# wendongbi/Bridged-GNN

Hardware: AMD Instinct MI355X
Metric: aggregated_edges_per_sec_ktgnn_fwd (higher is better)
Workload: dtype f32; 1 GPU; C4 synthetic bridged graph (local) N=1000000 E'=20991058, 2-layer KT-GNN eval fwd F=128 hidden=128 C=2; parallelism=single, execution=eager launches

## Files before the change

bridged_gnn_amd/_lib.py:

```python
import ctypes as C
import os

import torch

_HERE = os.path.dirname(os.path.abspath(__file__))
SO_PATH = os.path.join(_HERE, "csrc", "libbgnn_hip.so")
_lib = None

_P, _I64, _I32, _F32, _SZ, _INT = C.c_void_p, C.c_int64, C.c_int32, C.c_float, C.c_size_t, C.c_int

SIGNATURES = {
    "bgnn_version": (_INT, []),
    "bgnn_source_hash": (C.c_char_p, []),
    "bgnn_error_string": (C.c_char_p, [_INT]),
    "bgnn_csr_workspace_bytes": (_SZ, [_I64, _I64]),
    "bgnn_build_dst_csr": (_INT, [_P, _I64, _I64, _INT, _P, _P, _P, _P, _P, _SZ, _P]),
    "bgnn_domain_sums_f64": (_INT, [_P, _I64, _I32, _I64, _P, _P, _P]),
    "bgnn_domain_sums_workspace_bytes": (_SZ, [_I32]),
    "bgnn_domain_sums_ws_f64": (_INT, [_P, _I64, _I32, _I64, _P, _P, _P, _SZ, _P]),
    "bgnn_domain_delta_f32": (_INT, [_P, _I32, _P, _P]),
    "bgnn_adaptedconv_transform_f32": (_INT, [_P, _I64, _I32, _I64, _P, _P, _P, _I32, _I32, _P, _P, _P, _P,
                                               _P, _P, _P, _P, _I64, _I64, _I64, _I64, _P, _P, _I32, _P, _P]),
    "bgnn_classifier_stage_f32": (_INT, [_P, _I64, _I32, _I64, _P, _P, _I32, _I32, _P, _P, _P, _P, _P, _P, _P, _P, _I64, _I64,
                                          _P, _P, _I32, _INT, _P, _P, _P, _P, _P, _P]),
# ... 4 lines not shown
    "bgnn_narrow_transform_finish_rows32_f32": (_INT, [_P, _I64, _P, _P, _I32, _P, _P, _P, _P, _P, _P, _I64, _P, _P]),
    "bgnn_adaptedconv_aggregate_heads_rows32_plan": (_INT, [_P, _P, _I64, _I64, _I32, _F32]),
    "bgnn_adaptedconv_aggregate_heads_rows32_f32": (_INT, [_P, _P, _P, _P, _P, _P, _P, _I64, _I64, _I32, _F32, _P, _INT, _I64, _P]),
    "bgnn_gram_workspace_bytes": (C.c_size_t, [_I32, _I32]),
    "bgnn_gram_f32": (_INT, [_P, _I64, _I32, _P, _I64, _I32, _I64, _P, _P, C.c_size_t, _P]),
    "bgnn_transform_bwd_prep_workspace_bytes": (C.c_size_t, [_I64, _I32]),
    "bgnn_transform_bwd_prep_f32": (_INT, [_P, _I64, _I64, _I32, _P, _P, _I64, _I32, _P, _P, _P, _P, _P, _P, _I32, _I64, _P, _I64, _P, _P, C.c_size_t, _P]),
    "bgnn_bn_acc_doubles": (_I64, [_I32]),
    "bgnn_bn_relu_dropout_f32": (_INT, [_P, _I64, _I32, _I64, _P, _P, _F32, _INT, _F32, C.c_uint64, _P, _F32, _P, _P, _P, _I64, _P, _P]),
    "bgnn_bn_relu_dropout_bwd_f32": (_INT, [_P, _P, _I64, _I32, _I64, _I64, _P, _P, _P, _F32, _INT, _F32, C.c_uint64, _P, _P, _I64, _P, _P]),
    "bgnn_bn_colstats_f32": (_INT, [_P, _I64, _I32, _I64, _P, _P]),
    "bgnn_bn_apply_rows_f32": (_INT, [_P, _I64, _I32, _I64, _P, _I64, _P, _P, _F32, _INT, _F32, C.c_uint64, _P, _P, _I64, _F32, _P, _P, _P, _I64, _P]),
    "bgnn_bn_bwd_reduce_rows_f32": (_INT, [_P, _P, _I64, _I32, _I64, _I64, _P, _I64, _P, _P, _F32, _INT, _F32, C.c_uint64, _P, _P, _I64, _P, _P]),
    "bgnn_bn_bwd_apply_rows_f32": (_INT, [_P, _P, _I64, _I32, _I64, _I64, _P, _P, _I64, _P, _P, _F32, _INT, _F32, C.c_uint64, _P, _P, _I64, _P, _I64, _P]),
    "bgnn_transform_bwd_consts_f32": (_INT, [_P, _P, _P, _P, _P, _I32, _I32, _P, _P, _P, _P]),
    "bgnn_transform_bwd_finish_f32": (_INT, [_P, _P, _P, _P, _P, _P, _P, _I32, _I32, _I32, _P, _P, _P, _P, _P, _P, _P, _I64, _P]),
    "bgnn_rowdot_f32": (_INT, [_P, _I64, _I64, _I32, _P, _I64, _I32, _P, _P]),
    "bgnn_linear_f32": (_INT, [_P, _I64, _I32, _I64, _P, _P, _I32, _INT, _P, _P, _P, _I64, _P]),
    "bgnn_adaptedconv_aggregate_f32": (_INT, [_P, _P, _I64, _P, _P, _P, _P, _P, _I64, _I64, _I32, _F32,
                                               _P, _I64, _P, _P, _P, _INT, _P, _INT, _I64, _I32, _P, _P, _P]),
    "bgnn_adaptedconv_aggregate_bounded_f32": (_INT, [_P, _P, _I64, _P, _P, _P, _P, _P, _I64, _I64, _I32, _F32,
                                                       _P, _I64, _P, _P, _P, _INT, _P, _INT, _I64, _I32, _P, _P, _I64, _I32, _P]),
    "bgnn_aggregate_tile_queue_words": (_I64, []),
    "bgnn_adaptedconv_aggregate_queued_f32": (_INT, [_P, _P, _I64, _P, _P, _P, _P, _P, _I64, _I64, _I32, _F32,
                                                      _P, _I64, _P, _P, _P, _INT, _P, _INT, _I64, _I32, _P, _P, _I64, _I64, _I32, _P]),
    "bgnn_aggregate_hub_workspace_bytes": (C.c_size_t, [_I64, _I32, _I64]),
    "bgnn_adaptedconv_aggregate_hub_f32": (_INT, [_P, _P, _I64, _P, _P, _P, _P, _P, _I64, _I32, _F32, _P, _I64, _P, _P, _INT, _P, _I32, _P,
                                                   _P, _I32, _P, _I64, _P, _P, _P, _I64, _P, _P, C.c_size_t, _P]),
    "bgnn_adaptedconv_aggregate_bwd_f32": (_INT, [_P, _P, _I64, _P, _P, _P, _P, _P, _I64, _I64, _I32, _F32,
                                                   _P, _I64, _P, _P, _I64, _P, _P, _P, _P, _P]),
    "bgnn_aggregate_bwd_pull_workspace_bytes": (C.c_size_t, [_I64, _I64, _I64, _I32, _I64, _I64]),
    "bgnn_adaptedconv_aggregate_bwd_pull_f32": (_INT, [_P, _P, _I64, _P, _P, _P, _P, _P, _P, _P, _P, _I64, _I64, _I32, _F32,
                                                        _P, _I64, _P, _P, _I64, _P, _P, _P, _P, _I32,
                                                        _P, _I64, _P, _P, _P, _I64, _P, _I64, _P, _P, _P, _I64, _P, C.c_size_t, _P]),
    "bgnn_aggregate_heads_bwd_workspace_bytes": (C.c_size_t, [_I64, _I64, _I32, _I64, _I64]),
    "bgnn_adaptedconv_aggregate_heads_bwd_f32": (_INT, [_P, _P, _P, _P, _P, _P, _P, _P, _P, _I64, _I64, _I32, _I32, _F32,
                                                         _P, _P, _P, _INT, _P, _P, _P, _P, _I32,
                                                         _P, _I64, _P, _P, _P, _I64, _P, _I64, _P, _P, _P, _I64, _P, C.c_size_t, _P]),
    "bgnn_adaptedconv_aggregate_heads_wide_f32": (_INT, [_P, _P, _I64, _P, _P, _P, _P, _P, _I64, _I32, _I32, _F32, _P, _P, _P]),
    "bgnn_aggregate_heads_wide_bwd_workspace_bytes": (C.c_size_t, [_I64, _I32, _I64]),
    "bgnn_adaptedconv_aggregate_heads_wide_bwd_f32": (_INT, [_P, _P, _I64, _P, _P, _P, _P, _P, _P, _P, _I64, _I32, _I32, _F32,
                                                              _P, _P, _P, _P, _P, _P, _P, _P, C.c_size_t, _P]),
    "bgnn_l2_normalize_rows_f32": (_INT, [_P, _I64, _I32, _F32, _P, _P]),
    "bgnn_topk_workspace_bytes": (_SZ, [_I64, _I64, _I32]),
    "bgnn_cosine_topk_f32": (_INT, [_P, _P, _I64, _I64, _I32, _I32, _INT, _P, _P, _P, _P, _SZ, _P]),
    "bgnn_mlp_pair_topk_f32": (_INT, [_P, _P, _P, _P, _P, _F32, _I64, _I64, _I32, _I32, _INT, _P, _P, _P,
# ... 210 lines not shown
```

bridged_gnn_amd/csrc/bgnn_aggregate.hip:

```cpp
#include <cstdlib>
#include <cstring>
#include <type_traits>
#include "bgnn_common.h"

namespace {

struct AggParams {
  const float* h_t2s;
  const float* h_s2t;
  int64_t ldh;
  const float* a_t2s;
  const float* a_s2t;
  const int32_t* rowptr;
  const int32_t* col;
  const uint8_t* mask;
  int64_t row_begin;
  int64_t row_end;
  int32_t D;
  float slope;
  float* out;
  int64_t ldo;
  float* alpha;
  const float* ep_scale;
  const float* ep_shift;
// ... 479 lines not shown
  }
  if (p.colsum != nullptr) {
    unsafeAtomicAdd(&red[0][f0], cs_s.x); unsafeAtomicAdd(&red[0][f0 + 1], cs_s.y);
    unsafeAtomicAdd(&red[0][f0 + 2], cs_s.z); unsafeAtomicAdd(&red[0][f0 + 3], cs_s.w);
    unsafeAtomicAdd(&red[1][f0], cs_t.x); unsafeAtomicAdd(&red[1][f0 + 1], cs_t.y);
    unsafeAtomicAdd(&red[1][f0 + 2], cs_t.z); unsafeAtomicAdd(&red[1][f0 + 3], cs_t.w);
    if (lg == 0) { unsafeAtomicAdd(&red[0][LF * 4], n_s); unsafeAtomicAdd(&red[1][LF * 4], n_t); }
    __syncthreads();
    for (int t = threadIdx.x; t < 2 * (LF * 4 + 1); t += 256) {
      const int d = t / (LF * 4 + 1), c = t % (LF * 4 + 1);
      const double sum = (double)red[d][c];
      if (c == LF * 4) unsafeAtomicAdd(&p.colsum[2 * p.ldo + d], sum);
      else if (c < p.ldo) unsafeAtomicAdd(&p.colsum[d * p.ldo + c], sum);
    }
  }
}

typedef unsigned int u32x4_t __attribute__((ext_vector_type(4)));
constexpr int TQ_SPACING_WORDS = 32;

template <int CTRL>
__device__ __forceinline__ uint32_t dpp_movu(uint32_t x) { return (uint32_t)__builtin_amdgcn_update_dpp(0, (int)x, CTRL, 0xF, 0xF, true); }

template <int LF, bool ALPHA>
__global__ __launch_bounds__(256) void agg_wide_fast_kernel(AggParams p) {
  static_assert(LF == 16 || LF == 32 || LF == 64, "wide rows only");
  constexpr int U = 4;
  constexpr int GPW = 64 / LF;
  constexpr int RPB = 4 * GPW;
  const int lane = threadIdx.x & 63;
  const int wave = threadIdx.x >> 6;
  const int g = lane / LF;
  const int lg = lane % LF;
  const int f0 = lg * 4;
  const bool fvalid = f0 < p.D;
  const int f0c = fvalid ? f0 : 0;
  const int k = lane & (U - 1);
  const bool b0 = lane & 1, b1 = lane & 2;

  const int32_t row0 = (int32_t)p.row_begin, row1 = (int32_t)p.row_end;
  const int32_t ntiles = (row1 - row0 + RPB - 1) / RPB;
  __shared__ float red[2][LF * 4 + 1];
  __shared__ unsigned long long cl_ring[4];
  __shared__ uint32_t cl_prog[4];
  const bool tile_claims = p.tile_queue != nullptr && p.tq_subqueues > 0;
  if (tile_claims && threadIdx.x < 4) { cl_ring[threadIdx.x] = 0ull; cl_prog[threadIdx.x] = 0u; }
  if (p.colsum != nullptr)
    for (int t = threadIdx.x; t < 2 * (LF * 4 + 1); t += 256) (&red[0][0])[t] = 0.f;
  if (p.colsum != nullptr || tile_claims) __syncthreads();
  __shared__ unsigned int dyn_tile;
  const uint32_t nstride = (uint32_t)(p.ldh * 4);
  const uint32_t ostride = (uint32_t)(p.ldo * 4);
  const __amdgpu_buffer_rsrc_t rt = __builtin_amdgcn_make_buffer_rsrc(const_cast<char*>(p.tbl_base), (short)0, (int)p.tbl_bytes, 0x00020000);
  const __amdgpu_buffer_rsrc_t ro = __builtin_amdgcn_make_buffer_rsrc(p.out, (short)0, (int)((uint32_t)row1 * ostride), 0x00020000);
  const f2 sl = {p.slope, p.slope};
  float sc4[4] = {0.f, 0.f, 0.f, 0.f}, sh4[4] = {0.f, 0.f, 0.f, 0.f};
  if (p.ep_scale != nullptr) {
#pragma unroll
    for (int c = 0; c < 4; ++c)
      if (f0 + c < p.D) { sc4[c] = p.ep_scale[f0 + c]; sh4[c] = p.ep_shift[f0 + c]; }
  }
  f2 cs_s01 = {0.f, 0.f}, cs_s23 = cs_s01, cs_t01 = cs_s01, cs_t23 = cs_s01;
  float n_s = 0.f, n_t = 0.f;
  f2 aS01 = {0.f, 0.f}, aS23 = aS01, aT01 = aS01, aT23 = aS01;
  if (fvalid) {
    aS01.x = p.a_t2s[f0]; aS01.y = f0 + 1 < p.D ? p.a_t2s[f0 + 1] : 0.f;
    aS23.x = f0 + 2 < p.D ? p.a_t2s[f0 + 2] : 0.f; aS23.y = f0 + 3 < p.D ? p.a_t2s[f0 + 3] : 0.f;
    aT01.x = p.a_s2t[f0]; aT01.y = f0 + 1 < p.D ? p.a_s2t[f0 + 1] : 0.f;
    aT23.x = f0 + 2 < p.D ? p.a_s2t[f0 + 2] : 0.f; aT23.y = f0 + 3 < p.D ? p.a_s2t[f0 + 3] : 0.f;
  }
  const int32_t TQ_CHUNK = p.tq_chunk;
  const int32_t xcd = blockIdx.x % 8, slot = blockIdx.x / 8;
  const int32_t G = ((int32_t)gridDim.x + 7 - xcd) / 8;
  const int32_t tstride = p.tq_interleave ? G : 1;
  const int32_t NSEG = p.xcd_segments > 1 ? p.xcd_segments : 1;
  const int32_t per_x = (ntiles + 7) / 8, seg_len = (per_x + NSEG - 1) / NSEG;
  const int32_t xbase = xcd * per_x;
  const int32_t xend = NSEG > 1 ? xbase + NSEG * seg_len : min((xcd + 1) * per_x, ntiles);
  int32_t tile = xbase + slot - G;
  int32_t chunk_left = 0;
  const int32_t NQ = tile_claims ? min((int32_t)p.tq_subqueues, G) : 0;
  const int32_t wave_u = __builtin_amdgcn_readfirstlane(wave);
  uint32_t* const qctr = NQ > 0 ? p.tile_queue + (xcd * NQ + slot % NQ) * TQ_SPACING_WORDS : nullptr;
  const int32_t qpos0 = xbase + (NQ > 0 ? slot % NQ : 0);
  uint32_t cl_n = 0;
  uint32_t cl_val = 0;
  bool cl_own = false, cl_pending = false;
  bool cl_ending = false, cl_stop = false;
  auto cl_issue = [&](uint32_t& v) {
    uint64_t ex;
    asm volatile("s_mov_b64 %1, exec\n\ts_mov_b64 exec, 1\n\tglobal_atomic_add %0, %2, %3, %4 sc0\n\ts_mov_b64 exec, %1"
                 : "+v"(v), "=&s"(ex) : "v"(0u), "v"(1u), "s"(qctr) : "memory");
  };
// ... 63 lines not shown
      if (tile >= xend) break;
    }
    int32_t gt = tile;
    if (NSEG > 1) {
      const int32_t j = tile - xbase, sg = j / seg_len;
      gt = (sg * 8 + xcd) * seg_len + (j - sg * seg_len);
      if (gt >= ntiles) {
        if (cl_own) {
          uint32_t v = 0;
          cl_issue(v);
          cl_wait(v);
          cl_publish(cl_n + 1u, v);
        }
        continue;
      }
    }
    const int32_t i0 = row0 + gt * RPB + wave * GPW + g;
    const bool rvalid = i0 < row1;
    const int32_t ic = rvalid ? i0 : row0;
    const bool dom_s = p.mask[ic] != 0;
    const int32_t beg = rvalid ? p.rowptr[ic] : 0;
    const int32_t end = rvalid ? p.rowptr[ic + 1] : 0;
    const uint32_t lbase = (dom_s ? p.off_t2s : p.off_s2t) + (uint32_t)f0c * 4u;
    const f2 a01 = dom_s ? aS01 : aT01, a23 = dom_s ? aS23 : aT23;
    const float4 hi4 = __builtin_bit_cast(float4, __builtin_amdgcn_raw_buffer_load_b128(rt, lbase + __umul24((uint32_t)ic, nstride), 0, 0));
    f2 h01 = {hi4.x, hi4.y}, h23 = {hi4.z, hi4.w};

    float m = -INFINITY, s = 0.f;
    f2 acc01 = {0.f, 0.f}, acc23 = {0.f, 0.f};
    const int32_t niter = (end - beg + U - 1) / U;
    auto issue = [&](float4 (&v)[U], uint32_t off) {
      v[0] = __builtin_bit_cast(float4, __builtin_amdgcn_raw_buffer_load_b128(rt, lbase + dpp_movu<0x00>(off), 0, 0));
      v[1] = __builtin_bit_cast(float4, __builtin_amdgcn_raw_buffer_load_b128(rt, lbase + dpp_movu<0x55>(off), 0, 0));
      v[2] = __builtin_bit_cast(float4, __builtin_amdgcn_raw_buffer_load_b128(rt, lbase + dpp_movu<0xAA>(off), 0, 0));
      v[3] = __builtin_bit_cast(float4, __builtin_amdgcn_raw_buffer_load_b128(rt, lbase + dpp_movu<0xFF>(off), 0, 0));
      asm volatile("" : "+v"(h01), "+v"(h23) : : "memory");
      __builtin_amdgcn_sched_barrier(0);
    };
    auto take_id = [&](uint32_t& id) {
      __builtin_amdgcn_sched_barrier(0);
      asm volatile("s_waitcnt vmcnt(0)" : "+v"(id), "+v"(m), "+v"(s), "+v"(acc01), "+v"(acc23) : : "memory");
    };
    auto load_id = [&](int32_t ee) {
      uint32_t id;
      const uint32_t eoff = (uint32_t)max(min(ee, end - 1), 0) * 4u;
      __builtin_amdgcn_sched_barrier(0);
      asm volatile("global_load_dword %0, %1, %2" : "=v"(id) : "v"(eoff), "s"(p.col) : "memory");
      __builtin_amdgcn_sched_barrier(0);
      return id;
    };
    auto row_off = [&](uint32_t id, bool alive) { return alive ? __umul24(id, nstride) : p.dead_off; };
    auto update = [&](const float4 (&v)[U], bool ok, int32_t e_cur) {
      float t[U];
#pragma unroll
      for (int u = 0; u < U; ++u) {
        f2 z0 = f2{v[u].x, v[u].y} + h01, z1 = f2{v[u].z, v[u].w} + h23;
        z0 = __builtin_elementwise_max(z0, z0 * sl);
        z1 = __builtin_elementwise_max(z1, z1 * sl);
        f2 q = a01 * z0;
        q = __builtin_elementwise_fma(a23, z1, q);
        t[u] = q.x + q.y;
      }
      const float rA = bfly<0xB1>(b0, t[0], t[1]), rB = bfly<0xB1>(b0, t[2], t[3]);
      float r = bfly<0x4E>(b1, rA, rB);
// ... 16 lines not shown
#define BGNN_ACC(u, w)                                               \
      {                                                              \
        acc01.x = fmaf(w, v[u].x, acc01.x); acc01.y = fmaf(w, v[u].y, acc01.y); \
        acc23.x = fmaf(w, v[u].z, acc23.x); acc23.y = fmaf(w, v[u].w, acc23.y); \
      }
#ifdef AGGF_X_NOACC
      acc01.x += pe * v[0].x + v[1].y + v[2].z + v[3].w;
#else
      { const float w = quad_bcast<0>(pe); BGNN_ACC(0, w) }
      { const float w = quad_bcast<1>(pe); BGNN_ACC(1, w) }
      { const float w = quad_bcast<2>(pe); BGNN_ACC(2, w) }
      { const float w = quad_bcast<3>(pe); BGNN_ACC(3, w) }
#endif
#undef BGNN_ACC
      m = mn;
    };
    int32_t nw = __builtin_amdgcn_readlane(niter, 0);
    if constexpr (LF <= 32) nw = max(nw, __builtin_amdgcn_readlane(niter, 32));
    if constexpr (LF <= 16) nw = max(nw, max(__builtin_amdgcn_readlane(niter, 16), __builtin_amdgcn_readlane(niter, 48)));
    int32_t e = beg + k;
    bool ok = e < end;
    uint32_t myoff = p.dead_off;
    if (nw > 0) myoff = row_off((uint32_t)p.col[max(min(e, end - 1), 0)], ok);
    asm volatile("" : "+v"(h01), "+v"(h23) : : "memory");
    if (cl_own) {
      cl_issue(cl_val);
      if (p.tq_ahead) cl_pending = true;
      else { cl_wait(cl_val); cl_publish(cl_n + 1u, cl_val); }
    }
    for (int32_t it = 0; it < nw; ++it) {
      float4 v[U];
      issue(v, myoff);
      const int32_t e_cur = e;
      e += U;
      const bool ok2 = e < end;
      uint32_t nextid = load_id(e);
      update(v, ok, e_cur);
      ok = ok2;
      take_id(nextid);
      if (cl_pending) {
        asm volatile("" : "+v"(cl_val) : : "memory");
        cl_publish(cl_n + 1u, cl_val);
        cl_pending = false;
        __builtin_amdgcn_sched_barrier(0);
      }
      myoff = row_off(nextid, ok);
    }
    if (cl_pending) {
      cl_wait(cl_val);
      cl_publish(cl_n + 1u, cl_val);
      cl_pending = false;
    }
    s += bgnn::dpp_mov<0xB1>(s);
    s += bgnn::dpp_mov<0x4E>(s);

    const float inv = 1.f / (s + 1e-16f);
    if constexpr (ALPHA) {
      if (lg < U) {
        for (int32_t e2 = beg + lg; e2 < end; e2 += 4 * U) {
          float a[4];
#pragma unroll
          for (int j = 0; j < 4; ++j) a[j] = e2 + j * U < end ? p.alpha[e2 + j * U] : 0.f;
#pragma unroll
          for (int j = 0; j < 4; ++j)
            if (e2 + j * U < end) p.alpha[e2 + j * U] = __expf(a[j] - m) * inv;
        }
      }
    }
    if (rvalid && f0 < p.ldo) {
      float4 o = make_float4(acc01.x * inv, acc01.y * inv, acc23.x * inv, acc23.y * inv);
      if (p.ep_scale != nullptr) {
        o.x = fmaf(o.x, sc4[0], sh4[0]); o.y = fmaf(o.y, sc4[1], sh4[1]);
        o.z = fmaf(o.z, sc4[2], sh4[2]); o.w = fmaf(o.w, sc4[3], sh4[3]);
      }
      if (p.ep_relu) { o.x = fmaxf(o.x, 0.f); o.y = fmaxf(o.y, 0.f); o.z = fmaxf(o.z, 0.f); o.w = fmaxf(o.w, 0.f); }
      if (!fvalid) o = make_float4(0.f, 0.f, 0.f, 0.f);
      __builtin_amdgcn_raw_buffer_store_b128(__builtin_bit_cast(u32x4_t, o), ro, __umul24((uint32_t)i0, ostride) + (uint32_t)f0 * 4u, 0, 0);
      if (p.colsum != nullptr) {
        const float ws = dom_s ? 1.f : 0.f, wt = dom_s ? 0.f : 1.f;
        const f2 ws2 = {ws, ws}, wt2 = {wt, wt}, o01 = {o.x, o.y}, o23 = {o.z, o.w};
        cs_s01 = __builtin_elementwise_fma(o01, ws2, cs_s01); cs_s23 = __builtin_elementwise_fma(o23, ws2, cs_s23);
        cs_t01 = __builtin_elementwise_fma(o01, wt2, cs_t01); cs_t23 = __builtin_elementwise_fma(o23, wt2, cs_t23);
        n_s += ws; n_t += wt;
      }
    }
  }
  if (p.colsum != nullptr) {
    unsafeAtomicAdd(&red[0][f0], cs_s01.x); unsafeAtomicAdd(&red[0][f0 + 1], cs_s01.y);
    unsafeAtomicAdd(&red[0][f0 + 2], cs_s23.x); unsafeAtomicAdd(&red[0][f0 + 3], cs_s23.y);
    unsafeAtomicAdd(&red[1][f0], cs_t01.x); unsafeAtomicAdd(&red[1][f0 + 1], cs_t01.y);
    unsafeAtomicAdd(&red[1][f0 + 2], cs_t23.x); unsafeAtomicAdd(&red[1][f0 + 3], cs_t23.y);
    if (lg == 0) { unsafeAtomicAdd(&red[0][LF * 4], n_s); unsafeAtomicAdd(&red[1][LF * 4], n_t); }
    __syncthreads();
    for (int t = threadIdx.x; t < 2 * (LF * 4 + 1); t += 256) {
      const int d = t / (LF * 4 + 1), c = t % (LF * 4 + 1);
      const double sum = (double)red[d][c];
      if (c == LF * 4) unsafeAtomicAdd(&p.colsum[2 * p.ldo + d], sum);
      else if (c < p.ldo) unsafeAtomicAdd(&p.colsum[d * p.ldo + c], sum);
    }
  }
}

template <int HEADS, int EP, int U>
__global__ __launch_bounds__(256) void agg_heads_lanes_kernel(AggParams p) {
  constexpr int GL = EP * HEADS, GPW = 64 / GL, RPB = 4 * GPW;
  const int lane = threadIdx.x & 63, wave = threadIdx.x >> 6;
  const int g = lane / GL, lg = lane % GL;
  const int sub = lg / HEADS, h = lg % HEADS;
  const bool lane_on = g < GPW;
  const int64_t ntiles = (p.row_end - p.row_begin + p.n_vrows + RPB - 1) / RPB;
  bgnn::XcdRange tr = bgnn::xcd_pos_range(ntiles);
  const int64_t rs = (int64_t)HEADS * p.ldh;
  for (int64_t pos = tr.begin; pos < tr.end; pos += tr.step) {
    const int64_t tile = bgnn::xcd_tile_of(pos, ntiles);
    if (tile < 0) continue;
// ... 600 lines not shown
  if (span > lim32 || p.row_end * rs > lim32) return false;
  p.tbl_base = lo;
  p.tbl_bytes = (uint32_t)span;
  p.off_t2s = (uint32_t)(a - lo);
  p.off_s2t = (uint32_t)(b - lo);
  p.dead_off = (uint32_t)span;
  return true;
}

constexpr int kClaimTileDefault = 1;
struct ClaimCfg { int tile, nq, ahead; };
static const ClaimCfg& claim_cfg() {
  static const ClaimCfg c = [] {
    ClaimCfg r{kClaimTileDefault, 4, 1};
    if (const char* e = getenv("BGNN_AGG_CLAIM")) r.tile = strcmp(e, "chunk") == 0 ? 0 : (strcmp(e, "tile") == 0 ? 1 : r.tile);
    if (const char* e = getenv("BGNN_AGG_SUBQUEUES")) { const int v = atoi(e); if (v >= 1 && v <= 8) r.nq = v; }
    if (const char* e = getenv("BGNN_AGG_CLAIM_AHEAD")) r.ahead = atoi(e) != 0;
    return r;
  }();
  return c;
}
static int64_t claim_queue_words() { return (int64_t)8 * claim_cfg().nq * TQ_SPACING_WORDS; }

template <int LF, bool ALPHA>
int launch_wide_fast(const AggParams& p, hipStream_t st) {
  constexpr int RPB = 4 * (64 / LF);
  static const int per_cu_max = [] {
    int per_cu = 0;
    if (hipOccupancyMaxActiveBlocksPerMultiprocessor(&per_cu, agg_wide_fast_kernel<LF, ALPHA>, 256, 0) != hipSuccess || per_cu < 1) return 0;
    if (per_cu > 8) per_cu = 8;
    const char* e = getenv("BGNN_AGG_BLOCKS_PER_CU");
    if (e && atoi(e) > 0 && atoi(e) < per_cu) per_cu = atoi(e);
    return per_cu;
  }();
  static const int n_cu = [] {
    int dev = 0;
    hipDeviceProp_t prop;
    if (hipGetDevice(&dev) != hipSuccess || hipGetDeviceProperties(&prop, dev) != hipSuccess) return 0;
    return prop.multiProcessorCount;
  }();
  static const bool forced = getenv("BGNN_AGG_BLOCKS_PER_CU") != nullptr;
  int per_cu = per_cu_max;
  if (p.gather_hint == 2 && !forced && per_cu > 3) per_cu = 3;
  const int64_t cap = (per_cu_max > 0 && n_cu > 0) ? (int64_t)per_cu * n_cu / 8 * 8 : 2048;
  const int64_t ntiles = (p.row_end - p.row_begin + RPB - 1) / RPB;
  int64_t grid = ntiles < cap ? (ntiles + 7) / 8 * 8 : cap;
  if (grid < 8) grid = 8;
  AggParams q = p;
  q.tq_chunk = tq_chunk_for(ntiles, grid);
  static const int il = [] { const char* e = getenv("BGNN_AGG_INTERLEAVE"); return e ? atoi(e) : 1; }();
  q.tq_interleave = il;
  static const int nseg = [] { const char* e = getenv("BGNN_XCD_SEGMENTS"); return e ? atoi(e) : 8; }();
  q.xcd_segments = nseg;
  const ClaimCfg& cc = claim_cfg();
  const bool tile_claims = cc.tile && p.tile_queue != nullptr && p.tq_words >= claim_queue_words();
  q.tq_subqueues = tile_claims ? cc.nq : 0;
  q.tq_ahead = cc.ahead;
  hipLaunchKernelGGL((agg_wide_fast_kernel<LF, ALPHA>), dim3((unsigned)grid), dim3(256), 0, st, q);
  BGNN_LAUNCH_CHECK();
  return 0;
}

struct HubMergeParams {
  const int32_t* hub_rows; const int32_t* seg_ptr; int64_t n_hubs;
  const float* part_acc;
  const float* part_ms;
  const uint8_t* mask;
  int32_t D; int64_t ldo; int32_t heads;
  float* out; const float* ep_scale; const float* ep_shift; int ep_relu;
  double* colsum; float* state_ms;
  float* alpha; const int32_t* rowptr;
};

template <int LF>
__global__ __launch_bounds__(256) void hub_merge_wide_kernel(HubMergeParams p) {
  const int lane = threadIdx.x % LF, grp = threadIdx.x / LF;
  constexpr int GPB = 256 / LF;
  const int f0 = lane * 4;
  const bool fvalid = f0 < p.D;
  __shared__ float red[2][LF * 4 + 1];
  if (p.colsum != nullptr) {
    for (int t = threadIdx.x; t < 2 * (LF * 4 + 1); t += 256) (&red[0][0])[t] = 0.f;
    __syncthreads();
// ... 260 lines not shown
                out, 4, nullptr, nullptr, nullptr, ep_relu, nullptr, nullptr, 3, nullptr, 0, row_begin, 4};
  return heads_fast_plan(p, table_rows, true) ? 0 : BGNN_E_SHAPE;
}

extern "C" int bgnn_adaptedconv_aggregate_heads_rows32_plan(const float* t_t2s, const float* t_s2t, int64_t table_rows,
                                                            int64_t row_end, int32_t D, float negative_slope) {
  AggParams p;
  return rows32_params(p, t_t2s, t_s2t, nullptr, nullptr, nullptr, nullptr, nullptr, 0, row_end, D, negative_slope, nullptr, 0, table_rows) == 0;
}

extern "C" int bgnn_adaptedconv_aggregate_heads_rows32_f32(const float* t_t2s, const float* t_s2t, const float* a_t2s, const float* a_s2t,
                                                           const int32_t* rowptr, const int32_t* col, const uint8_t* mask,
                                                           int64_t row_begin, int64_t row_end, int32_t D, float negative_slope,
                                                           float* out, int ep_relu, int64_t table_rows, void* stream) {
  if (!a_t2s || !a_s2t || !rowptr || !col || !mask || !out) return BGNN_E_NULL;
  AggParams p;
  const int rc = rows32_params(p, t_t2s, t_s2t, a_t2s, a_s2t, rowptr, col, mask, row_begin, row_end, D, negative_slope, out, ep_relu, table_rows);
  if (rc) return rc;
  if (row_end == row_begin) return 0;
  return launch_heads_rows32(p, (hipStream_t)stream);
}

extern "C" int64_t bgnn_aggregate_tile_queue_words(void) { return claim_cfg().tile ? claim_queue_words() : 8; }

extern "C" int bgnn_adaptedconv_aggregate_queued_f32(const float* h_t2s, const float* h_s2t, int64_t ldh,
                                                     const float* a_t2s, const float* a_s2t,
                                                     const int32_t* rowptr, const int32_t* col, const uint8_t* mask,
                                                     int64_t row_begin, int64_t row_end, int32_t D, float negative_slope,
                                                     float* out, int64_t ldo, float* alpha_opt,
                                                     const float* ep_scale_opt, const float* ep_shift_opt, int ep_relu,
                                                     float* state_ms_opt, int part, int64_t park_begin, int32_t heads,
                                                     double* colsum_opt, uint32_t* tile_queue_opt, int64_t tile_queue_words,
                                                     int64_t table_rows, int32_t gather_hint, void* stream) {
  if (table_rows < row_end || gather_hint < 0 || gather_hint > 2) return BGNN_E_SHAPE;
  return aggregate_impl(h_t2s, h_s2t, ldh, a_t2s, a_s2t, rowptr, col, mask, row_begin, row_end, D, negative_slope, out, ldo, alpha_opt,
                        ep_scale_opt, ep_shift_opt, ep_relu, state_ms_opt, part, park_begin, heads, colsum_opt, tile_queue_opt,
                        tile_queue_words, table_rows, gather_hint, stream);
}

extern "C" size_t bgnn_aggregate_hub_workspace_bytes(int64_t n_segments, int32_t heads, int64_t ldo) {
  const size_t nv = (size_t)(n_segments > 0 ? n_segments : 0), h = (size_t)(heads > 0 ? heads : 1);
  return bgnn_align_up(sizeof(float) * nv * h * (size_t)(ldo > 0 ? ldo : 0), 256) + bgnn_align_up(sizeof(float) * 2 * nv * h, 256) + 256;
}

extern "C" int bgnn_adaptedconv_aggregate_hub_f32(const float* h_t2s, const float* h_s2t, int64_t ldh,
                                                  const float* a_t2s, const float* a_s2t,
// ... 98 lines not shown
```

bridged_gnn_amd/ops.py:

```python
import ctypes
import os

import torch

from . import _lib as L

__all__ = ["DstCSR", "build_dst_csr", "domain_delta", "pack_transform_heads", "adaptedconv_transform", "adaptedconv_aggregate", "linear", "linear_supported", "linear_narrow_supported", "linear_narrow_transform", "narrow_transform_finish", "gram", "gram_supported", "rowdot", "transform_bwd_prep", "topk_edges_coalesced",
           "l2_normalize_rows", "cosine_topk", "mlp_pair_topk", "topk_edges", "coalesce", "gather_rows", "pad4",
           "sage_mean_aggregate", "sage_mean_aggregate_bwd", "rows_segment_add", "gcn_aggregate", "gcn_aggregate_bwd", "gat_scores", "gat_aggregate", "gat_aggregate_bwd", "gatv2_aggregate", "gatv2_aggregate_bwd", "wide_heads_supported",
           "adaptedconv_aggregate_heads_wide", "adaptedconv_aggregate_heads_wide_bwd", "pair_csr", "pair_mlp_stats", "pair_mlp_loss",
           "pair_mlp_segsum", "pair_mlp_eval", "pair_mlp_count", "PAIR_MLP_WIDTH", "pair_cos_loss", "pair_cos_segsum", "pair_cos_count",
           "PAIR_COS_WIDTH"]


def pad4(n):
    return (int(n) + 3) // 4 * 4


HUB_THRESHOLD = 128
HUB_SEGMENT = 64


class DstCSR:

# ... 525 lines not shown
    if delta is None and H == 1 and (tile_need is not None or tail_single[0] or tail_single[1]):
        c = getattr(tile_need, "_team_plan", None)
        runs = c[1] if (c is not None and c[0] == (N, dev, tile_need._version)) else transform_team_runs(N, dev, tile_need, tail_single)
    flat = (ctypes.c_int64 * (3 * len(runs)))(*[v for r in runs for v in r]) if runs else None
    rc = lib.bgnn_adaptedconv_transform_f32(
        L.ptr(x), N, Din, x.stride(0), L.ptr(mask_u8), L.ptr(delta), None if delta is not None else L.ptr(sums), H, D, L.ptr(Wp), L.ptr(bp),
        L.ptr(gates), L.ptr(gconst), L.ptr_rows(out[0][1]), L.ptr_rows(out[0][0]), L.ptr_rows(o1[1]), L.ptr_rows(o1[0]), ldh, row_stride,
        int(tail_single[0]), int(tail_single[1]), L.ptr(tile_need), flat, len(runs), L.ptr(small), L.stream())
    L.check(rc, "bgnn_adaptedconv_transform_f32")
    return out


_P2_STATIC = os.environ.get("BGNN_P2_STATIC", "1") != "0"


_TILE_QUEUE_WORDS = None


def _tile_queue(dev):
    global _TILE_QUEUE_WORDS
    if _TILE_QUEUE_WORDS is None:
        _TILE_QUEUE_WORDS = max(8, int(L.lib().bgnn_aggregate_tile_queue_words()))
    return torch.empty(_TILE_QUEUE_WORDS, dtype=torch.int32, device=dev)


def heads_log_softmax_supported(heads, D):
    return heads in (2, 3) and D <= 4


def _hub_shape_ok(D, ldh, ldo, heads, slope):
    if heads in (2, 3) and D <= 4 and ldh == 4 and ldo == 4:
        return True
    return heads == 1 and D > 32 and 0.0 <= slope <= 1.0


def adaptedconv_aggregate(h_t2s, h_s2t, a_t2s, a_s2t, csr, mask_u8, D, negative_slope=0.1, n_dst=None,
                          want_alpha=False, ep_scale=None, ep_shift=None, ep_relu=False, out=None,
                          row_begin=0, row_end=None, state_ms=None, part=0, heads=1, colsum=None, log_softmax=False,
                          park_begin=None):
    lib = L.lib()
    n_dst = csr.num_nodes if n_dst is None else int(n_dst)
    row_end = n_dst if row_end is None else int(row_end)
    ldh = h_t2s.stride(0) // heads
    ldo = pad4(D)
    dev = h_t2s.device
    if out is None:
# ... 1661 lines not shown
```

include/bgnn.h:

```cpp
#ifndef BGNN_H_
#define BGNN_H_
#include <stddef.h>
#include <stdint.h>

#ifdef __cplusplus
extern "C" {
#endif

#define BGNN_VERSION 116
#define BGNN_E_NULL (-1)
#define BGNN_E_SHAPE (-2)
#define BGNN_E_WORKSPACE (-3)
#define BGNN_E_ALIGN (-4)
#define BGNN_E_RANGE (-5)

int bgnn_version(void);
const char* bgnn_error_string(int code);
const char* bgnn_source_hash(void);

size_t bgnn_csr_workspace_bytes(int64_t N, int64_t E);
int bgnn_build_dst_csr(const int64_t* edge_index, int64_t E, int64_t N, int rewrite_self_loops,
                       int32_t* rowptr, int32_t* col, int32_t* eperm_opt, int64_t* E_out_dev,
                       void* ws, size_t ws_bytes, void* stream);

// ... 85 lines not shown
                                   int64_t ldh, int64_t row_stride, int64_t n_tail_t2s, int64_t n_tail_s2t,
                                   const int32_t* tile_need_opt, const int64_t* team_runs_host_opt, int32_t n_team_runs,
                                   float* small_ws, void* stream);

int bgnn_adaptedconv_aggregate_f32(const float* h_t2s, const float* h_s2t, int64_t ldh,
                                   const float* a_t2s, const float* a_s2t,
                                   const int32_t* rowptr, const int32_t* col, const uint8_t* mask,
                                   int64_t row_begin, int64_t row_end, int32_t D, float negative_slope,
                                   float* out, int64_t ldo, float* alpha_opt,
                                   const float* ep_scale_opt, const float* ep_shift_opt, int ep_relu,
                                   float* state_ms_opt, int part, int64_t park_begin, int32_t heads, double* colsum_opt,
                                   uint32_t* tile_queue_opt, void* stream);

int bgnn_adaptedconv_aggregate_bounded_f32(const float* h_t2s, const float* h_s2t, int64_t ldh,
                                           const float* a_t2s, const float* a_s2t,
                                           const int32_t* rowptr, const int32_t* col, const uint8_t* mask,
                                           int64_t row_begin, int64_t row_end, int32_t D, float negative_slope,
                                           float* out, int64_t ldo, float* alpha_opt,
                                           const float* ep_scale_opt, const float* ep_shift_opt, int ep_relu,
                                           float* state_ms_opt, int part, int64_t park_begin, int32_t heads, double* colsum_opt,
                                           uint32_t* tile_queue_opt, int64_t table_rows, int32_t gather_hint, void* stream);

int64_t bgnn_aggregate_tile_queue_words(void);
int bgnn_adaptedconv_aggregate_queued_f32(const float* h_t2s, const float* h_s2t, int64_t ldh,
                                          const float* a_t2s, const float* a_s2t,
                                          const int32_t* rowptr, const int32_t* col, const uint8_t* mask,
                                          int64_t row_begin, int64_t row_end, int32_t D, float negative_slope,
                                          float* out, int64_t ldo, float* alpha_opt,
                                          const float* ep_scale_opt, const float* ep_shift_opt, int ep_relu,
                                          float* state_ms_opt, int part, int64_t park_begin, int32_t heads, double* colsum_opt,
                                          uint32_t* tile_queue_opt, int64_t tile_queue_words, int64_t table_rows, int32_t gather_hint,
                                          void* stream);

size_t bgnn_aggregate_hub_workspace_bytes(int64_t n_segments, int32_t heads, int64_t ldo);
int bgnn_adaptedconv_aggregate_hub_f32(const float* h_t2s, const float* h_s2t, int64_t ldh,
                                       const float* a_t2s, const float* a_s2t,
                                       const int32_t* rowptr, const int32_t* col, const uint8_t* mask,
                                       int64_t N, int32_t D, float negative_slope, float* out, int64_t ldo,
                                       const float* ep_scale_opt, const float* ep_shift_opt, int ep_relu,
                                       float* state_ms_opt, int32_t heads, double* colsum_opt,
                                       uint32_t* tile_queue_opt, int32_t hub_threshold, const int32_t* hub_rows,
                                       int64_t n_hubs, const int32_t* hub_seg_ptr, const int32_t* seg_bounds,
                                       const int32_t* seg_node, int64_t n_segments, float* alpha_opt,
                                       void* ws, size_t ws_bytes, void* stream);

int bgnn_adaptedconv_aggregate_bwd_f32(const float* h_t2s, const float* h_s2t, int64_t ldh,
// ... 301 lines not shown
```

Before: 55.84 billion edges/s.

## Move wide aggregate constants and colsum accumulators to LDS, cap blocks per CU

The wide aggregation kernel now keeps the epilogue scale/shift and attention vectors in shared memory instead of per-thread registers, and accumulates per-lane column sums in LDS rather than register accumulators. This is meant to lower register pressure and allow higher occupancy. Blocks per CU are capped at 5 or 6 by default. An optional double-buffered gather that prefetches two steps ahead is added behind an environment variable, but it is off by default. The cost is extra LDS traffic and LDS read-modify-writes per output row.

After: 55.27 billion edges/s. 0.99x the previous value.

```diff
diff --git a/bridged_gnn_amd/_lib.py b/bridged_gnn_amd/_lib.py
--- a/bridged_gnn_amd/_lib.py
+++ b/bridged_gnn_amd/_lib.py
@@ -50,6 +50,7 @@
     "bgnn_adaptedconv_aggregate_bounded_f32": (_INT, [_P, _P, _I64, _P, _P, _P, _P, _P, _I64, _I64, _I32, _F32,
                                                        _P, _I64, _P, _P, _P, _INT, _P, _INT, _I64, _I32, _P, _P, _I64, _I32, _P]),
     "bgnn_aggregate_tile_queue_words": (_I64, []),
+    "bgnn_aggregate_wide_fast_blocks_per_cu": (_INT, [_INT, _INT]),
     "bgnn_adaptedconv_aggregate_queued_f32": (_INT, [_P, _P, _I64, _P, _P, _P, _P, _P, _I64, _I64, _I32, _F32,
                                                       _P, _I64, _P, _P, _P, _INT, _P, _INT, _I64, _I32, _P, _P, _I64, _I64, _I32, _P]),
     "bgnn_aggregate_hub_workspace_bytes": (C.c_size_t, [_I64, _I32, _I64]),
diff --git a/bridged_gnn_amd/csrc/bgnn_aggregate.hip b/bridged_gnn_amd/csrc/bgnn_aggregate.hip
--- a/bridged_gnn_amd/csrc/bgnn_aggregate.hip
+++ b/bridged_gnn_amd/csrc/bgnn_aggregate.hip
@@ -525,7 +525,7 @@
 template <int CTRL>
 __device__ __forceinline__ uint32_t dpp_movu(uint32_t x) { return (uint32_t)__builtin_amdgcn_update_dpp(0, (int)x, CTRL, 0xF, 0xF, true); }
 
-template <int LF, bool ALPHA>
+template <int LF, bool ALPHA, int AHEAD>
 __global__ __launch_bounds__(256) void agg_wide_fast_kernel(AggParams p) {
   static_assert(LF == 16 || LF == 32 || LF == 64, "wide rows only");
   constexpr int U = 4;
@@ -550,28 +550,27 @@
   if (tile_claims && threadIdx.x < 4) { cl_ring[threadIdx.x] = 0ull; cl_prog[threadIdx.x] = 0u; }
   if (p.colsum != nullptr)
     for (int t = threadIdx.x; t < 2 * (LF * 4 + 1); t += 256) (&red[0][0])[t] = 0.f;
-  if (p.colsum != nullptr || tile_claims) __syncthreads();
+  __shared__ __attribute__((aligned(16))) float cst[4][LF * 4];
+  __shared__ float4 cs_lane[2][256];
+  __shared__ float cs_rows[2][256 / LF];
+  if (p.colsum != nullptr) {
+    cs_lane[0][threadIdx.x] = cs_lane[1][threadIdx.x] = make_float4(0.f, 0.f, 0.f, 0.f);
+    if (threadIdx.x < 2 * (256 / LF)) (&cs_rows[0][0])[threadIdx.x] = 0.f;
+  }
+  for (int c = threadIdx.x; c < LF * 4; c += 256) {
+    const bool in = c < p.D;
+    cst[0][c] = in && p.ep_scale != nullptr ? p.ep_scale[c] : 0.f;
+    cst[1][c] = in && p.ep_scale != nullptr ? p.ep_shift[c] : 0.f;
+    cst[2][c] = in ? p.a_t2s[c] : 0.f;
+    cst[3][c] = in ? p.a_s2t[c] : 0.f;
+  }
+  __syncthreads();
   __shared__ unsigned int dyn_tile;
   const uint32_t nstride = (uint32_t)(p.ldh * 4);
   const uint32_t ostride = (uint32_t)(p.ldo * 4);
   const __amdgpu_buffer_rsrc_t rt = __builtin_amdgcn_make_buffer_rsrc(const_cast<char*>(p.tbl_base), (short)0, (int)p.tbl_bytes, 0x00020000);
   const __amdgpu_buffer_rsrc_t ro = __builtin_amdgcn_make_buffer_rsrc(p.out, (short)0, (int)((uint32_t)row1 * ostride), 0x00020000);
   const f2 sl = {p.slope, p.slope};
-  float sc4[4] = {0.f, 0.f, 0.f, 0.f}, sh4[4] = {0.f, 0.f, 0.f, 0.f};
-  if (p.ep_scale != nullptr) {
-#pragma unroll
-    for (int c = 0; c < 4; ++c)
-      if (f0 + c < p.D) { sc4[c] = p.ep_scale[f0 + c]; sh4[c] = p.ep_shift[f0 + c]; }
-  }
-  f2 cs_s01 = {0.f, 0.f}, cs_s23 = cs_s01, cs_t01 = cs_s01, cs_t23 = cs_s01;
-  float n_s = 0.f, n_t = 0.f;
-  f2 aS01 = {0.f, 0.f}, aS23 = aS01, aT01 = aS01, aT23 = aS01;
-  if (fvalid) {
-    aS01.x = p.a_t2s[f0]; aS01.y = f0 + 1 < p.D ? p.a_t2s[f0 + 1] : 0.f;
-    aS23.x = f0 + 2 < p.D ? p.a_t2s[f0 + 2] : 0.f; aS23.y = f0 + 3 < p.D ? p.a_t2s[f0 + 3] : 0.f;
-    aT01.x = p.a_s2t[f0]; aT01.y = f0 + 1 < p.D ? p.a_s2t[f0 + 1] : 0.f;
-    aT23.x = f0 + 2 < p.D ? p.a_s2t[f0 + 2] : 0.f; aT23.y = f0 + 3 < p.D ? p.a_s2t[f0 + 3] : 0.f;
-  }
   const int32_t TQ_CHUNK = p.tq_chunk;
   const int32_t xcd = blockIdx.x % 8, slot = blockIdx.x / 8;
   const int32_t G = ((int32_t)gridDim.x + 7 - xcd) / 8;
@@ -681,7 +680,8 @@
     const int32_t beg = rvalid ? p.rowptr[ic] : 0;
     const int32_t end = rvalid ? p.rowptr[ic + 1] : 0;
     const uint32_t lbase = (dom_s ? p.off_t2s : p.off_s2t) + (uint32_t)f0c * 4u;
-    const f2 a01 = dom_s ? aS01 : aT01, a23 = dom_s ? aS23 : aT23;
+    const float4 a4 = *reinterpret_cast<const float4*>(&cst[dom_s ? 2 : 3][f0]);
+    f2 a01 = {a4.x, a4.y}, a23 = {a4.z, a4.w};
     const float4 hi4 = __builtin_bit_cast(float4, __builtin_amdgcn_raw_buffer_load_b128(rt, lbase + __umul24((uint32_t)ic, nstride), 0, 0));
     f2 h01 = {hi4.x, hi4.y}, h23 = {hi4.z, hi4.w};
 
@@ -698,7 +698,7 @@
     };
     auto take_id = [&](uint32_t& id) {
       __builtin_amdgcn_sched_barrier(0);
-      asm volatile("s_waitcnt vmcnt(0)" : "+v"(id), "+v"(m), "+v"(s), "+v"(acc01), "+v"(acc23) : : "memory");
+      asm volatile("s_waitcnt vmcnt(%5)" : "+v"(id), "+v"(m), "+v"(s), "+v"(acc01), "+v"(acc23) : "n"(AHEAD == 2 ? U : 0) : "memory");
     };
     auto load_id = [&](int32_t ee) {
       uint32_t id;
@@ -761,12 +761,45 @@
     bool ok = e < end;
     uint32_t myoff = p.dead_off;
     if (nw > 0) myoff = row_off((uint32_t)p.col[max(min(e, end - 1), 0)], ok);
-    asm volatile("" : "+v"(h01), "+v"(h23) : : "memory");
+    bool okn = e + U < end;
+    uint32_t offn = p.dead_off;
+    if constexpr (AHEAD == 2) {
+      if (nw > 0) offn = row_off((uint32_t)p.col[max(min(e + U, end - 1), 0)], okn);
+    }
+    asm volatile("" : "+v"(h01), "+v"(h23), "+v"(a01), "+v"(a23) : : "memory");
     if (cl_own) {
       cl_issue(cl_val);
       if (p.tq_ahead) cl_pending = true;
       else { cl_wait(cl_val); cl_publish(cl_n + 1u, cl_val); }
     }
+    if constexpr (AHEAD == 2) {
+      if (nw > 0) {
+        float4 vA[U], vB[U];
+        issue(vA, myoff);
+        uint32_t idn = 0;
+        if (nw > 2) idn = load_id(e + 2 * U);
+        auto step = [&](const float4 (&cur)[U], float4 (&nxt)[U], int32_t it) {
+          issue(nxt, offn);
+          const int32_t e_cur = e;
+          e += U;
+          update(cur, ok, e_cur);
+          ok = okn;
+          take_id(idn);
+          if (cl_pending) {
+            asm volatile("" : "+v"(cl_val) : : "memory");
+            cl_publish(cl_n + 1u, cl_val);
+            cl_pending = false;
+            __builtin_amdgcn_sched_barrier(0);
+          }
+          okn = e + U < end;
+          offn = row_off(idn, okn);
+          if (it + 3 < nw) idn = load_id(e + 2 * U);
+        };
+        int32_t it = 0;
+        for (; it + 1 < nw; it += 2) { step(vA, vB, it); step(vB, vA, it + 1); }
+        if (it < nw) step(vA, vB, it);
+      }
+    } else
     for (int32_t it = 0; it < nw; ++it) {
       float4 v[U];
       issue(v, myoff);
@@ -809,27 +842,30 @@
     if (rvalid && f0 < p.ldo) {
       float4 o = make_float4(acc01.x * inv, acc01.y * inv, acc23.x * inv, acc23.y * inv);
       if (p.ep_scale != nullptr) {
-        o.x = fmaf(o.x, sc4[0], sh4[0]); o.y = fmaf(o.y, sc4[1], sh4[1]);
-        o.z = fmaf(o.z, sc4[2], sh4[2]); o.w = fmaf(o.w, sc4[3], sh4[3]);
+        const float4 sc4 = *reinterpret_cast<const float4*>(&cst[0][f0]), sh4 = *reinterpret_cast<const float4*>(&cst[1][f0]);
+        o.x = fmaf(o.x, sc4.x, sh4.x); o.y = fmaf(o.y, sc4.y, sh4.y);
+        o.z = fmaf(o.z, sc4.z, sh4.z); o.w = fmaf(o.w, sc4.w, sh4.w);
       }
       if (p.ep_relu) { o.x = fmaxf(o.x, 0.f); o.y = fmaxf(o.y, 0.f); o.z = fmaxf(o.z, 0.f); o.w = fmaxf(o.w, 0.f); }
       if (!fvalid) o = make_float4(0.f, 0.f, 0.f, 0.f);
       __builtin_amdgcn_raw_buffer_store_b128(__builtin_bit_cast(u32x4_t, o), ro, __umul24((uint32_t)i0, ostride) + (uint32_t)f0 * 4u, 0, 0);
       if (p.colsum != nullptr) {
-        const float ws = dom_s ? 1.f : 0.f, wt = dom_s ? 0.f : 1.f;
-        const f2 ws2 = {ws, ws}, wt2 = {wt, wt}, o01 = {o.x, o.y}, o23 = {o.z, o.w};
-        cs_s01 = __builtin_elementwise_fma(o01, ws2, cs_s01); cs_s23 = __builtin_elementwise_fma(o23, ws2, cs_s23);
-        cs_t01 = __builtin_elementwise_fma(o01, wt2, cs_t01); cs_t23 = __builtin_elementwise_fma(o23, wt2, cs_t23);
-        n_s += ws; n_t += wt;
+        float4& cs = cs_lane[dom_s ? 0 : 1][threadIdx.x];
+        float4 c4 = cs;
+        c4.x += o.x; c4.y += o.y; c4.z += o.z; c4.w += o.w;
+        cs = c4;
+        if (lg == 0) cs_rows[dom_s ? 0 : 1][threadIdx.x / LF] += 1.f;
       }
     }
   }
   if (p.colsum != nullptr) {
-    unsafeAtomicAdd(&red[0][f0], cs_s01.x); unsafeAtomicAdd(&red[0][f0 + 1], cs_s01.y);
-    unsafeAtomicAdd(&red[0][f0 + 2], cs_s23.x); unsafeAtomicAdd(&red[0][f0 + 3], cs_s23.y);
-    unsafeAtomicAdd(&red[1][f0], cs_t01.x); unsafeAtomicAdd(&red[1][f0 + 1], cs_t01.y);
-    unsafeAtomicAdd(&red[1][f0 + 2], cs_t23.x); unsafeAtomicAdd(&red[1][f0 + 3], cs_t23.y);
-    if (lg == 0) { unsafeAtomicAdd(&red[0][LF * 4], n_s); unsafeAtomicAdd(&red[1][LF * 4], n_t); }
+#pragma unroll
+    for (int d = 0; d < 2; ++d) {
+      const float4 c4 = cs_lane[d][threadIdx.x];
+      unsafeAtomicAdd(&red[d][f0], c4.x); unsafeAtomicAdd(&red[d][f0 + 1], c4.y);
+      unsafeAtomicAdd(&red[d][f0 + 2], c4.z); unsafeAtomicAdd(&red[d][f0 + 3], c4.w);
+      if (lg == 0) unsafeAtomicAdd(&red[d][LF * 4], cs_rows[d][threadIdx.x / LF]);
+    }
     __syncthreads();
     for (int t = threadIdx.x; t < 2 * (LF * 4 + 1); t += 256) {
       const int d = t / (LF * 4 + 1), c = t % (LF * 4 + 1);
@@ -1476,17 +1512,30 @@
 }
 static int64_t claim_queue_words() { return (int64_t)8 * claim_cfg().nq * TQ_SPACING_WORDS; }
 
-template <int LF, bool ALPHA>
-int launch_wide_fast(const AggParams& p, hipStream_t st) {
-  constexpr int RPB = 4 * (64 / LF);
+constexpr int kStepsAheadDefault = 1;
+template <bool ALPHA> constexpr int kWideFastBlocksCap = ALPHA ? 5 : 6;
+static int steps_ahead() {
+  static const int a = [] { const char* e = getenv("BGNN_AGG_STEPS_AHEAD"); const int v = e ? atoi(e) : 0; return v == 1 || v == 2 ? v : kStepsAheadDefault; }();
+  return a;
+}
+
+template <int LF, bool ALPHA, int AHEAD>
+int wide_fast_per_cu() {
   static const int per_cu_max = [] {
     int per_cu = 0;
-    if (hipOccupancyMaxActiveBlocksPerMultiprocessor(&per_cu, agg_wide_fast_kernel<LF, ALPHA>, 256, 0) != hipSuccess || per_cu < 1) return 0;
+    if (hipOccupancyMaxActiveBlocksPerMultiprocessor(&per_cu, agg_wide_fast_kernel<LF, ALPHA, AHEAD>, 256, 0) != hipSuccess || per_cu < 1) return 0;
     if (per_cu > 8) per_cu = 8;
     const char* e = getenv("BGNN_AGG_BLOCKS_PER_CU");
-    if (e && atoi(e) > 0 && atoi(e) < per_cu) per_cu = atoi(e);
-    return per_cu;
+    if (e && atoi(e) > 0) return atoi(e) < per_cu ? atoi(e) : per_cu;
+    return per_cu > kWideFastBlocksCap<ALPHA> ? kWideFastBlocksCap<ALPHA> : per_cu;
   }();
+  return per_cu_max;
+}
+
+template <int LF, bool ALPHA, int AHEAD>
+int launch_wide_fast_ahead(const AggParams& p, hipStream_t st) {
+  constexpr int RPB = 4 * (64 / LF);
+  const int per_cu_max = wide_fast_per_cu<LF, ALPHA, AHEAD>();
   static const int n_cu = [] {
     int dev = 0;
     hipDeviceProp_t prop;
@@ -1510,9 +1559,27 @@
   const bool tile_claims = cc.tile && p.tile_queue != nullptr && p.tq_words >= claim_queue_words();
   q.tq_subqueues = tile_claims ? cc.nq : 0;
   q.tq_ahead = cc.ahead;
-  hipLaunchKernelGGL((agg_wide_fast_kernel<LF, ALPHA>), dim3((unsigned)grid), dim3(256), 0, st, q);
+  hipLaunchKernelGGL((agg_wide_fast_kernel<LF, ALPHA, AHEAD>), dim3((unsigned)grid), dim3(256), 0, st, q);
   BGNN_LAUNCH_CHECK();
   return 0;
+}
+
+template <int LF, bool ALPHA>
+int launch_wide_fast(const AggParams& p, hipStream_t st) {
+  return steps_ahead() == 2 ? launch_wide_fast_ahead<LF, ALPHA, 2>(p, st) : launch_wide_fast_ahead<LF, ALPHA, 1>(p, st);
+}
+
+static int wide_fast_blocks_per_cu(int D, int alpha) {
+  if (D <= 32 || D > 256 || (alpha != 0 && alpha != 1)) return BGNN_E_SHAPE;
+  const int nv = (D + 3) / 4, a2 = steps_ahead() == 2;
+  if (alpha) {
+    if (nv <= 16) return a2 ? wide_fast_per_cu<16, true, 2>() : wide_fast_per_cu<16, true, 1>();
+    if (nv <= 32) return a2 ? wide_fast_per_cu<32, true, 2>() : wide_fast_per_cu<32, true, 1>();
+    return a2 ? wide_fast_per_cu<64, true, 2>() : wide_fast_per_cu<64, true, 1>();
+  }
+  if (nv <= 16) return a2 ? wide_fast_per_cu<16, false, 2>() : wide_fast_per_cu<16, false, 1>();
+  if (nv <= 32) return a2 ? wide_fast_per_cu<32, false, 2>() : wide_fast_per_cu<32, false, 1>();
+  return a2 ? wide_fast_per_cu<64, false, 2>() : wide_fast_per_cu<64, false, 1>();
 }
 
 struct HubMergeParams {
@@ -1819,6 +1886,8 @@
 }
 
 extern "C" int64_t bgnn_aggregate_tile_queue_words(void) { return claim_cfg().tile ? claim_queue_words() : 8; }
+
+extern "C" int bgnn_aggregate_wide_fast_blocks_per_cu(int D, int alpha) { return wide_fast_blocks_per_cu(D, alpha); }
 
 extern "C" int bgnn_adaptedconv_aggregate_queued_f32(const float* h_t2s, const float* h_s2t, int64_t ldh,
                                                      const float* a_t2s, const float* a_s2t,
diff --git a/bridged_gnn_amd/ops.py b/bridged_gnn_amd/ops.py
--- a/bridged_gnn_amd/ops.py
+++ b/bridged_gnn_amd/ops.py
@@ -571,6 +571,13 @@
     if _TILE_QUEUE_WORDS is None:
         _TILE_QUEUE_WORDS = max(8, int(L.lib().bgnn_aggregate_tile_queue_words()))
     return torch.empty(_TILE_QUEUE_WORDS, dtype=torch.int32, device=dev)
+
+
+def aggregate_wide_fast_blocks_per_cu(D, alpha=False):
+    n = int(L.lib().bgnn_aggregate_wide_fast_blocks_per_cu(int(D), 1 if alpha else 0))
+    if n < 0:
+        raise ValueError(f"aggregate_wide_fast_blocks_per_cu: no wide kernel for D = {D}")
+    return n
 
 
 def heads_log_softmax_supported(heads, D):
diff --git a/include/bgnn.h b/include/bgnn.h
--- a/include/bgnn.h
+++ b/include/bgnn.h
@@ -131,6 +131,7 @@
                                            uint32_t* tile_queue_opt, int64_t table_rows, int32_t gather_hint, void* stream);
 
 int64_t bgnn_aggregate_tile_queue_words(void);
+int bgnn_aggregate_wide_fast_blocks_per_cu(int D, int alpha);
 int bgnn_adaptedconv_aggregate_queued_f32(const float* h_t2s, const float* h_s2t, int64_t ldh,
                                           const float* a_t2s, const float* a_s2t,
                                           const int32_t* rowptr, const int32_t* col, const uint8_t* mask,
```
